# facebookresearch/rela

Measured on AMD Instinct MI355X. Metric: env-steps/s (Ape-X Atari 84x84x4, actor tick + learner grad-step), higher is better.
Workload: dtype f32 (f32 operands as 3 exact bf16 parts on bf16 MFMA; f32-accurate); 1 GPU; Ape-X DQN 80x80 envs/GPU, actor+learner on one MI355X, replay 2^20, B=512, A=18, n=3; device-resident static frames; parallelism=single

## Files before the change

rela_amd/csrc/ffnet.hip:

```cpp
#include <atomic>
#include <cstdlib>

#include "common.h"
#include "gemm_bf16s.h"
#include "gemm_f32emu.h"
#include "gemm_s3.h"
#include "conv_img_s3.h"
#include "conv12_s3.h"
#include "ffnet_layout.h"
#include "ffnet_plan.h"
#include "gemm_lds.h"
#include "param_layout.h"
#include "prof.h"
#define RELA_WEIGHT_PACK_KERNEL
#include "weight_pack.h"

namespace rela_amd {

typedef float f32x4 __attribute__((ext_vector_type(4)));

struct FFNetDev {
  uint4* B1 = nullptr;
  float* b1 = nullptr;
  float *B2 = nullptr, *b2 = nullptr;
// ... 1869 lines not shown
int rela_amd::ffnet_load_extra(rela_ffnet* n, const rela_ffnet_params* p, void* stream_, const ExtraPacks& extra) {
  return ffnet_load_impl(n, p, 1, stream_, extra);
}

int rela_amd::ffnet_load_impl(rela_ffnet* n, const rela_ffnet_params* p, int on_device, void* stream_,
                              const ExtraPacks& extra) {
  RELA_CHECK(n && p, RELA_EINVAL, "rela_ffnet_load: bad arguments");
  hipStream_t s = (hipStream_t)stream_;
  DeviceGuard g(n->device);
  const int A = n->num_action;
  int64_t cnt[kFFNetSegs];
  ffnet_param_counts(A, cnt);
  const float* src[12] = {p->conv1_w, p->conv1_b, p->conv2_w, p->conv2_b, p->conv3_w, p->conv3_b,
                          p->fc_w,    p->fc_b,    p->v_w,     p->v_b,     p->a_w,     p->a_b};
  const float* dv[12];
  float* tmp = nullptr;
  if (int rc = stage_params(src, cnt, 12, on_device, "rela_ffnet_load", &tmp, dv, s)) return rc;
  const uint32_t set = ffnet_pack_set(n->max_rows, n->precision, on_device != 0);
  n->bft_src = ffnet_bft_on_demand(n->max_rows, n->precision, on_device != 0) ? dv[6] : nullptr;
  if (int rc = pack_layouts(n->d, set, dv, 12, A, extra, dv[6], s)) return rc;
  n->packed = set;
  if (int rc = free_staging(tmp, s)) return rc;
  n->loaded = true;
  n->version += 1;
  return RELA_OK;
}

extern "C" int rela_ffnet_forward(const rela_ffnet* n, int N, const uint8_t* s_dev, const float* legal_dev,
                                  float* q_dev, void* ws, int64_t ws_bytes, void* stream_) {
  return rela_amd::ffnet_forward_mode(n, N, s_dev, legal_dev, q_dev, ws, ws_bytes, stream_, kModeNet);
}

int rela_amd::ffnet_forward_mode(const rela_ffnet* n, int N, const uint8_t* s_dev, const float* legal_dev, float* q_dev,
                                 void* ws, int64_t ws_bytes, void* stream_, int mode, int rows_limit) {
  RELA_CHECK(n && n->loaded, RELA_ESTATE, "rela_ffnet_forward: parameters were never loaded");
  const int max_rows = rows_limit < 0 ? n->max_rows : rows_limit;
  RELA_CHECK(N >= 1 && s_dev && legal_dev && q_dev && ws, RELA_EINVAL, "rela_ffnet_forward: bad arguments");
  RELA_CHECK(ws_bytes >= rela_ffnet_workspace_bytes(n, N), RELA_EINVAL,
             "rela_ffnet_forward: workspace of %lld bytes is too small for batch %d", (long long)ws_bytes, N);
  RELA_CHECK(((uintptr_t)s_dev & 15) == 0 && ((uintptr_t)ws & 15) == 0, RELA_EINVAL,
             "rela_ffnet_forward: s_dev and workspace must be 16-byte aligned");
  RELA_CHECK(max_rows <= 0 || N <= max_rows, RELA_EINVAL,
             "rela_ffnet_forward: batch %d on a net whose owner declared at most %d rows", N, max_rows);
  hipStream_t s = (hipStream_t)stream_;
  const FFNetWs w = ffnet_ws(ws, N);
  const FFNetDev& d = n->d;
  const char* const* names = n->prof_names ? n->prof_names : kProfActor;
  const char* name12 = n->prof_names ? "learner_fwd_conv12" : "conv12_fused";
  const FfnetPlan plan = plan_ffnet_forward(mode, n->precision, N, max_rows);
  uint32_t missing = ffnet_plan_reads(plan) & ~n->packed;
  if (missing == lay_bit(kLayBfT) && n->bft_src) {
    if (int rc = pack_one(kLayouts[kLayBfT].kind, n->bft_src, nullptr, n->d.BfT, 0, 0, kLayouts[kLayBfT].elements, s)) return rc;
    n->packed |= lay_bit(kLayBfT);
    missing = 0;
  }
  RELA_CHECK(missing == 0, RELA_ESTATE,
             "rela_ffnet_forward: %d rows in mode %d read layouts (bits 0x%x) the net's last load did not pack (row limit %d)", N,
             plan.precision, missing, n->max_rows);

  uint8_t* rec2 = static_cast<uint8_t*>(ws) + ws_records_offset(N);
  uint8_t* rec3 = rec2 + (int64_t)N * kRec2Bytes;
  TrunkOpts opts;
  opts.keep_f32 = plan.keep_f32;
  opts.leave_a3_records = !plan.unsplit_a3;
  launch_trunk(d, plan.trunk, N, s_dev, w.a1, w.a2, w.a3, rec2, rec3, opts, {names[0], names[1], names[2], name12}, s);

  const uint8_t* a3_records = reinterpret_cast<const uint8_t*>(w.a3);
// ... 8 lines not shown
    case kFcBf16SplitK:
      launch_fc_bf16_splitk(d, a3_records, fc_part_ptr(ws, w.ha, N), w.h, N, names[3], s);
      break;
    case kFcS3:
    case kFcS3SplitK: {
      ProfScope prof(names[3], s);
      note_launch("gemm_s3<fc>");
      const s3::Plan pl = s3::plan<s3::ProbFc>(N, plan.fc == kFcS3SplitK);
      if (pl.slices > 1) {
        float* part = fc_part_ptr(ws, w.ha, N);
        s3::launch<s3::ProbFc, s3::kEpiRaw>(rec3, d.Bfe, d.bf, part, N, s, pl);
        launch_fc_reduce(part, pl.slices, N, d.bf, w.h, s);
      } else {
        s3::launch<s3::ProbFc, s3::kEpiRelu>(rec3, d.Bfe, d.bf, w.h, N, s);
      }
      break;
    }
    case kFcF32SplitK: {
      float* part = fc_part_ptr(ws, w.ha, N);
      ProbFcFwd p{};
      p.M = N, p.N = 512, p.K = 3136;
      p.a3 = w.a3, p.wt = d.BfT, p.part = part;
      gemm::launch_gemm<TileFcSmall>(p, plan.fc_slices, s, names[3]);
      launch_fc_reduce(part, plan.fc_slices, N, d.bf, w.h, s);
      break;
    }
    case kFcF32Gemm: {
      ProfScope prof(names[3], s);
      note_launch("gemm_mfma<GemmFc> (f32)");
      launch_gemm_bm<GemmFc, GemmFc112>(w.a3, nullptr, d.Bf, d.bf, w.h, nullptr, nullptr, N, s);
      break;
    }
  }
  if (plan.trunk == kTrunkS3 && plan.keep_f32) unsplit_s3_a23(rec2, rec3, w.a2, w.a3, N, s);
  {
    ProfScope prof(names[4], s);
    note_launch("heads_duel");
    hipLaunchKernelGGL(heads_duel, dim3(ceil_div(N, kHeadRows)), dim3(256), 0, s, (const float*)w.h, (const float*)d.Bhp,
                       (const float*)d.bh, legal_dev, w.ha, q_dev, N, n->num_action);
  }
  RELA_LAUNCH_CHECK();
  return RELA_OK;
}

namespace rela_amd {
namespace {
__global__ void unsplit_trunk_rows(uint8_t* __restrict__ a1, uint8_t* __restrict__ a2, uint8_t* __restrict__ a3, int rows,
                                   int blocks1, int blocks2) {
  int b = blockIdx.x;
  const int t = threadIdx.x;
  int64_t rec;
  int q, C;
  uint8_t* base;
  bool ok;
  if (b < blocks1) {
    rec = (int64_t)b * 32 + (t >> 3), q = t & 7, C = 32, base = a1, ok = rec < (int64_t)rows * 400;
  } else {
    b -= blocks1;
    base = a2;
    int64_t pixels = (int64_t)rows * 81;
    if (b >= blocks2) b -= blocks2, base = a3, pixels = (int64_t)rows * 49;
    rec = (int64_t)b * 16 + (t >> 4), q = t & 15, C = 64, ok = rec < pixels;
  }
  uint8_t* r = base + (ok ? rec : 0) * (C * 4);
  const uint2 hi = *reinterpret_cast<const uint2*>(r + q * 8), lo = *reinterpret_cast<const uint2*>(r + C * 2 + q * 8);
  float4 v;
  v.x = __uint_as_float(hi.x << 16) + __uint_as_float(lo.x << 16);
// ... 290 lines not shown
```

rela_amd/csrc/ffnet_layout.h:

```cpp
#pragma once
#include <hip/hip_runtime.h>

#include <cstdint>

namespace rela_amd {

constexpr int64_t kA1 = 400 * 32, kA2 = 81 * 64, kA3 = 49 * 64, kH = 512, kHA = 32;
constexpr int64_t kWsFloatsPerSample = kA1 + kA2 + kA3 + kH + kHA;
constexpr int64_t kRec2Bytes = 81 * 384, kRec3Bytes = 49 * 384;

struct FFNetWs {
  float *a1, *a2, *a3, *h, *ha;
};

inline FFNetWs ffnet_ws(void* ws, int N) {
  FFNetWs w;
  w.a1 = static_cast<float*>(ws);
  w.a2 = w.a1 + kA1 * N;
  w.a3 = w.a2 + kA2 * N;
  w.h = w.a3 + kA3 * N;
  w.ha = w.h + kH * N;
  return w;
}

enum { kPermConv2 = 0, kPermConv3 = 1, kPermFc = 2 };
constexpr int kPermFloats[3] = {64 * 512, 64 * 576, 512 * 3136};
__device__ __forceinline__ void permute_weight_at(int mode, int idx, const float* __restrict__ src, float* __restrict__ dst) {
  if (mode == kPermConv2) {
    const int oc = idx >> 9, n = idx & 511, c = n & 31, r = n >> 5;
    dst[idx] = src[((oc * 32 + c) * 4 + (r >> 2)) * 4 + (r & 3)];
  } else if (mode == kPermConv3) {
    const int oc = idx / 576, n = idx - oc * 576, c = n & 63, r = n >> 6;
    dst[idx] = src[((oc * 64 + c) * 3 + r / 3) * 3 + r % 3];
  } else {
    const int u = idx / 3136, n = idx - u * 3136, c = n & 63, pos = n >> 6;
    dst[idx] = src[(size_t)u * 3136 + c * 49 + pos];
  }
}
struct ExtraPacks {
  float *w2p = nullptr, *w3p = nullptr, *wfcp = nullptr;
};
}

#include "../../include/rela_amd.h"
namespace rela_amd {
int ffnet_load_extra(rela_ffnet* n, const rela_ffnet_params* p, void* stream, const ExtraPacks& extra);
int lstmnet_load_extra(rela_lstmnet* n, const rela_lstmnet_params* p, void* stream, const ExtraPacks& extra);
void ffnet_label_as_learner(rela_ffnet* n);
void ffnet_set_max_rows(rela_ffnet* n, int rows);
int ffnet_forward_mode(const rela_ffnet* n, int N, const uint8_t* s_dev, const float* legal_dev, float* q_dev, void* ws,
                       int64_t ws_bytes, void* stream, int mode, int rows_limit = -1);
bool ffnet_learner_forward_ok(const rela_ffnet* on, const rela_ffnet* tg, int B);
int ffnet_learner_forward(const rela_ffnet* on, const rela_ffnet* tg, int B, const uint8_t* s_obs, const uint8_t* s_next,
                          const float* legal, const float* nlegal, float* q_on, float* q_no, float* q_nt, void* ws_on,
                          void* ws_tg, int64_t ws_bytes, hipStream_t s);
int ffnet_learner_unsplit(int B, void* ws_on, hipStream_t s);

int lstmnet_trunk(const rela_lstmnet* n, int N, const uint8_t* s_dev, float* a1, float* a2, float* a3, hipStream_t s,
                  const char* const* names, bool fast = false, bool* a3_records = nullptr, uint8_t* s3_scratch = nullptr,
                  bool keep_f32 = true);
int64_t gate_x3_packed_bytes();
int pack_gate_x3(const float* w_ih_dev, void* dst, bool permuted, hipStream_t s);
int gate_x3_gemm(const uint8_t* a3_records, const void* packed, const float* bias, float* gx, int M, hipStream_t s);
int lstmnet_heads(const rela_lstmnet* n, int N, const float* o, const float* legal, float* ha, float* q, hipStream_t s,
                  const char* name);
int lstmnet_trunk_records(const rela_lstmnet* n, int N, const uint8_t* s_dev, float* a1, float* a2, float* a3, int a1_lo,
                          hipStream_t s, const char* const* names);
int trunk_unsplit_rows(float* a1, float* a2, float* a3, int rows, hipStream_t s);
}
```

rela_amd/csrc/gemm_bf16x3.h:

```cpp
#pragma once
#include <hip/hip_runtime.h>

#include <type_traits>

#include "common.h"
#include "gemm_lds.h"
#include "prof.h"

namespace rela_amd {
namespace gemm3 {

typedef float f32x4 __attribute__((ext_vector_type(4)));
typedef float f32x2 __attribute__((ext_vector_type(2)));
typedef __bf16 bf16x8 __attribute__((ext_vector_type(8)));
typedef __bf16 bf16x2 __attribute__((ext_vector_type(2)));
typedef short s16x4 __attribute__((ext_vector_type(4)));
typedef s16x4 __attribute__((address_space(3))) * lds_s16x4_ptr;

constexpr int kT = 512;
constexpr int BK = 32;

__device__ __forceinline__ int krow(int k) {
  const int g = k >> 3, j = k & 7;
  return j < 4 ? 4 * g + j : 16 + 4 * g + (j - 4);
// ... 62 lines not shown
  }
  const int xcd = blockIdx.x & 7, i = blockIdx.x >> 3;
  if (gm.mode == 1) {
    const int tiles = gm.gx * gm.gy;
    bz = (i / tiles) * 8 + xcd;
    const int t = i % tiles;
    bx = t % gm.gx, by = t / gm.gx;
    return bz < gm.gz;
  }
  bx = (i / gm.gy) * 8 + xcd, by = i % gm.gy, bz = 0;
  return bx < gm.gx;
}

template <class T, class P>
__global__ __launch_bounds__(kT) void gemm_bf16x3(const P p, const GridMap gm) {
  extern __shared__ __attribute__((aligned(16))) uint8_t smem[];
  int bx, by, bz;
  if (!grid_map(gm, bx, by, bz)) return;
  const int tid = threadIdx.x;
  const int wave = tid >> 6, lane = tid & 63;
  const int li = lane & 15, g = lane >> 4;
  const int wm = wave / T::WN, wn = wave % T::WN;
  const int bm0 = by * T::BM, bn0 = bx * T::BN;
  const int nch = (p.K + BK - 1) / BK;
  const int c0 = bz * p.kslice;
  const int c1 = min(nch, c0 + p.kslice);
  constexpr int S = T::S;
  const int r0 = S == 1 ? c0 : 0, r1 = S == 1 ? c1 : (c1 - c0 + S - 1) / S;
  auto kbase = [&](int it, int sub) { return S == 1 ? it * BK : min(c0 + it * S + sub, c1 - 1) * BK; };

  constexpr int D = 4;
  typename P::StageA ra[D][T::A_IT];
  typename P::StageB rb[D][T::B_IT];
  auto gload = [&](int ch, auto set) {
    constexpr int R = decltype(set)::value;
    const int m0 = bm0, n0 = bn0;
#pragma unroll
    for (int j = 0; j < T::A_IT; ++j) {
      const int idx = min(tid + j * kT, T::A_V4 - 1);
      const int sub = idx / T::A_V4C, ic = idx % T::A_V4C;
      const int k0 = kbase(ch, sub);
      if constexpr (T::AMC) {
        const int kr = ic / (T::BM / 4), q = ic % (T::BM / 4);
        ra[R][j] = p.fetchA(k0 + kr, m0 + 4 * q);
      } else {
        const int r = ic >> 3, q = ic & 7;
        ra[R][j] = p.fetchA(m0 + r, k0 + 4 * q);
      }
    }
#pragma unroll
    for (int j = 0; j < T::B_IT; ++j) {
      const int idx = min(tid + j * kT, T::B_V4 - 1);
      const int sub = idx / T::B_V4C, ic = idx % T::B_V4C;
      const int kr = ic / (T::BN / 4), q = ic % (T::BN / 4);
      rb[R][j] = p.fetchB(kbase(ch, sub) + kr, n0 + 4 * q);
    }
  };
  auto sstore = [&](int buf, int ch, auto set) {
    constexpr int R = decltype(set)::value;
    const int z = gemm::store_point();
    const int m0 = bm0 + z, n0 = bn0 + z;
    uint8_t* base = smem + buf * T::BUF;
#pragma unroll
    for (int j = 0; j < T::A_IT; ++j) {
      const int idx = min(tid + j * kT, T::A_V4 - 1);
      const int sub = idx / T::A_V4C, ic = idx % T::A_V4C;
      const int k0 = kbase(ch, sub) + z;
      uint2 hi, mid, lo;
      float4 v;
      int off;
      if constexpr (T::AMC) {
        const int kr = ic / (T::BM / 4), q = ic % (T::BM / 4);
        v = p.fixA(ra[R][j], k0 + kr, m0 + 4 * q);
        off = sub * T::A_CHUNK + krow(kr) * T::LDA + q * 8;
      } else {
        const int r = ic >> 3, q = ic & 7;
        v = p.fixA(ra[R][j], m0 + r, k0 + 4 * q);
        off = sub * T::A_CHUNK + r * T::LDA + q * 8;
      }
      if constexpr (T::PARTS == 3) split4x3(v, hi, mid, lo);
      else split4(v, hi, lo);
      *reinterpret_cast<uint2*>(base + off) = hi;
      if constexpr (T::PARTS == 3) *reinterpret_cast<uint2*>(base + T::A_HALF + off) = mid;
      *reinterpret_cast<uint2*>(base + (T::PARTS - 1) * T::A_HALF + off) = lo;
    }
    uint8_t* bb = base + T::PARTS * T::A_HALF;
#pragma unroll
    for (int j = 0; j < T::B_IT; ++j) {
      const int idx = min(tid + j * kT, T::B_V4 - 1);
      const int sub = idx / T::B_V4C, ic = idx % T::B_V4C;
      const int kr = ic / (T::BN / 4), q = ic % (T::BN / 4);
      uint2 hi, mid, lo;
      const float4 v = p.fixB(rb[R][j], kbase(ch, sub) + z + kr, n0 + 4 * q);
      if constexpr (T::PARTS == 3) split4x3(v, hi, mid, lo);
      else split4(v, hi, lo);
      const int off = sub * T::B_CHUNK + krow(kr) * T::LDB + q * 8;
      *reinterpret_cast<uint2*>(bb + off) = hi;
      if constexpr (T::BPARTS == 3) *reinterpret_cast<uint2*>(bb + T::B_HALF + off) = mid;
      if constexpr (T::BPARTS > 1) *reinterpret_cast<uint2*>(bb + (T::BPARTS - 1) * T::B_HALF + off) = lo;
    }
  };

  const int tr_off = (4 * g + (li >> 2));
  auto frag_tr = [&](const uint8_t* img, int ld, int col0) -> bf16x8 {
    const uint8_t* a0 = img + tr_off * ld + (col0 + 4 * (li & 3)) * 2;
    const s16x4 x = __builtin_amdgcn_ds_read_tr16_b64_v4i16((lds_s16x4_ptr)(a0));
    const s16x4 y = __builtin_amdgcn_ds_read_tr16_b64_v4i16((lds_s16x4_ptr)(a0 + 16 * ld));
    typedef short s16x8 __attribute__((ext_vector_type(8)));
    const s16x8 z = {x[0], x[1], x[2], x[3], y[0], y[1], y[2], y[3]};
    return __builtin_bit_cast(bf16x8, z);
  };
  auto frag_row = [&](const uint8_t* img, int row) -> bf16x8 {
    return __builtin_bit_cast(bf16x8, *reinterpret_cast<const uint4*>(img + row * T::LDA + g * 16));
  };

  f32x4 acc[T::TM][T::TN];
  f32x4 accs[T::PARTS == 3 ? T::TM : 1][T::PARTS == 3 ? T::TN : 1];
#pragma unroll
  for (int t = 0; t < T::TM; ++t)
#pragma unroll
    for (int u = 0; u < T::TN; ++u) {
      acc[t][u] = f32x4{0.f, 0.f, 0.f, 0.f};
      if constexpr (T::PARTS == 3) accs[t][u] = f32x4{0.f, 0.f, 0.f, 0.f};
    }

  auto mma = [&](int buf, int ch, auto full) {
// ... 89 lines not shown
```

rela_amd/csrc/gemm_lds.h:

```cpp
#pragma once
#include <hip/hip_runtime.h>

#include <type_traits>
#include <utility>

#include "common.h"
#include "prof.h"

namespace rela_amd {
namespace gemm {

typedef float f32x4 __attribute__((ext_vector_type(4)));
constexpr int kLT = 512;
constexpr int BK = 32;

__device__ __forceinline__ float4 zero4() { return make_float4(0.f, 0.f, 0.f, 0.f); }
__device__ __forceinline__ float4 ld4(const float* p) { return *reinterpret_cast<const float4*>(p); }
__device__ __forceinline__ float4 keep4(bool in_range, float4 v) {
  return make_float4(in_range ? v.x : 0.f, in_range ? v.y : 0.f, in_range ? v.z : 0.f, in_range ? v.w : 0.f);
}

template <int BM_, int BN_, int WM_, int WN_, bool AMC_, int S_ = 1>
struct TileCfg {
  static constexpr int BM = BM_, BN = BN_, WM = WM_, WN = WN_, S = S_;
  static constexpr bool AMC = AMC_;
  static_assert(S == 1 || S == 2 || S == 4, "stage depth");
  static_assert(WM * WN == 8, "8 wavefronts per block");
  static constexpr int TM = BM / 16 / WM, TN = BN / 16 / WN;
  static_assert(TM >= 1 && TN >= 1, "tile too small for the wave grid");
  static constexpr int LDA = AMC ? BM + 16 : BK + 2;
  static constexpr int A_CHUNK = AMC ? BK * LDA : BM * LDA;
  static constexpr int A_FLOATS = S * A_CHUNK;
  static constexpr int LDB = BN + 16;
  static constexpr int B_CHUNK = BK * LDB;
  static constexpr int B_FLOATS = S * B_CHUNK;
  static constexpr int A_V4C = BM * BK / 4, B_V4C = BN * BK / 4;
  static constexpr int A_V4 = S * A_V4C, B_V4 = S * B_V4C;
  static constexpr int A_IT = (A_V4 + kLT - 1) / kLT, B_IT = (B_V4 + kLT - 1) / kLT;
  static constexpr int LDS_BYTES = 2 * (A_FLOATS + B_FLOATS) * 4;
  static constexpr bool DYN_LDS = LDS_BYTES > 64 * 1024;
};

template <class P, class = void>
struct fold_chunks {
  static constexpr int value = 0;
};
template <class P>
struct fold_chunks<P, std::void_t<decltype(P::kFoldChunks)>> {
  static constexpr int value = P::kFoldChunks;
};

__device__ __forceinline__ int store_point() {
  int z = 0;
  asm volatile("" : "+s"(z));
  return z;
}
template <class F, int... I>
__device__ __forceinline__ void static_for(F&& f, std::integer_sequence<int, I...>) {
  (f(std::integral_constant<int, I>{}), ...);
}
template <int D, class Load, class Store, class Mma>
__device__ __forceinline__ void chunk_ring(int c0, int c1, Load&& gload, Store&& sstore, Mma&& mma) {
  using Sets = std::make_integer_sequence<int, D>;
  static_for([&](auto j) { gload(min(c0 + j.value, c1 - 1), j); }, Sets{});
  sstore(0, c0, std::integral_constant<int, 0>{});
  __syncthreads();
  int base = c0;
  for (; base + D < c1; base += D) {
    static_for(
        [&](auto j) {
          const int cur = base + j.value, buf = (cur - c0) & 1;
          gload(min(cur + D, c1 - 1), j);
          __builtin_amdgcn_sched_barrier(0);
          mma(buf, cur, std::true_type{});
          __builtin_amdgcn_sched_barrier(0);
          sstore(buf ^ 1, cur + 1, std::integral_constant<int, (j.value + 1) % D>{});
          __syncthreads();
          __builtin_amdgcn_sched_barrier(0);
        },
        Sets{});
  }
  static_for(
      [&](auto j) {
// ... 6 lines not shown
      },
      Sets{});
}

constexpr int kRing = 2;

template <class T, class P>
__global__ __launch_bounds__(kLT) void gemm_lds(const P p) {
  constexpr int S = T::S;
  __shared__ __attribute__((aligned(16))) float sA_[2][T::DYN_LDS ? 4 : T::A_FLOATS];
  __shared__ __attribute__((aligned(16))) float sB_[2][T::DYN_LDS ? 4 : T::B_FLOATS];
  extern __shared__ __attribute__((aligned(16))) float gemm_lds_dyn[];
  auto pA = [&](int buf, int off) -> float* {
    if constexpr (T::DYN_LDS) return gemm_lds_dyn + buf * T::A_FLOATS + off;
    else return &sA_[buf][off];
  };
  auto pB = [&](int buf, int off) -> float* {
    if constexpr (T::DYN_LDS) return gemm_lds_dyn + (2 * T::A_FLOATS + buf * T::B_FLOATS) + off;
    else return &sB_[buf][off];
  };
  const int tid = threadIdx.x;
  const int wave = tid >> 6, lane = tid & 63;
  const int li = lane & 15, kk = lane >> 4;
  const int wm = wave / T::WN, wn = wave % T::WN;
  const int bm0 = blockIdx.y * T::BM, bn0 = blockIdx.x * T::BN;
  const int nch = (p.K + BK - 1) / BK;
  const int c0 = blockIdx.z * p.kslice;
  const int c1 = min(nch, c0 + p.kslice);
  const int r0 = S == 1 ? c0 : 0, r1 = S == 1 ? c1 : (c1 - c0 + S - 1) / S;
  auto kbase = [&](int it, int sub) { return S == 1 ? it * BK : min(c0 + it * S + sub, c1 - 1) * BK; };

  typename P::StageA ra[kRing][T::A_IT];
  typename P::StageB rb[kRing][T::B_IT];
  auto gload = [&](int ch, auto set) {
    constexpr int R = decltype(set)::value;
    const int m0 = bm0, n0 = bn0;
#pragma unroll
    for (int j = 0; j < T::A_IT; ++j) {
      const int idx = min(tid + j * kLT, T::A_V4 - 1);
      const int sub = S == 1 ? 0 : idx / T::A_V4C, ic = S == 1 ? idx : idx % T::A_V4C;
      const int k0 = kbase(ch, sub);
      if constexpr (T::AMC) {
        const int kr = ic / (T::BM / 4), q = ic % (T::BM / 4);
        ra[R][j] = p.fetchA(k0 + kr, m0 + 4 * q);
      } else {
        const int r = ic >> 3, q = ic & 7;
        ra[R][j] = p.fetchA(m0 + r, k0 + 4 * q);
      }
    }
#pragma unroll
    for (int j = 0; j < T::B_IT; ++j) {
      const int idx = min(tid + j * kLT, T::B_V4 - 1);
      const int sub = S == 1 ? 0 : idx / T::B_V4C, ic = S == 1 ? idx : idx % T::B_V4C;
      const int kr = ic / (T::BN / 4), q = ic % (T::BN / 4);
      rb[R][j] = p.fetchB(kbase(ch, sub) + kr, n0 + 4 * q);
    }
  };
  auto sstore = [&](int buf, int ch, auto set) {
    constexpr int R = decltype(set)::value;
    const int z = store_point();
    const int k00 = kbase(ch, 0) + z, m0 = bm0 + z, n0 = bn0 + z;
#pragma unroll
    for (int j = 0; j < T::A_IT; ++j) {
      const int idx = min(tid + j * kLT, T::A_V4 - 1);
      const int sub = S == 1 ? 0 : idx / T::A_V4C, ic = S == 1 ? idx : idx % T::A_V4C;
      const int k0 = S == 1 ? k00 : kbase(ch, sub) + z;
      if constexpr (T::AMC) {
        const int kr = ic / (T::BM / 4), q = ic % (T::BM / 4);
        *reinterpret_cast<float4*>(pA(buf, sub * T::A_CHUNK + kr * T::LDA + 4 * q)) = p.fixA(ra[R][j], k0 + kr, m0 + 4 * q);
      } else {
        const int r = ic >> 3, q = ic & 7;
        const float4 v = p.fixA(ra[R][j], m0 + r, k0 + 4 * q);
        float* d = pA(buf, sub * T::A_CHUNK + r * T::LDA + 4 * q);
        *reinterpret_cast<float2*>(d) = make_float2(v.x, v.y);
        *reinterpret_cast<float2*>(d + 2) = make_float2(v.z, v.w);
      }
    }
#pragma unroll
    for (int j = 0; j < T::B_IT; ++j) {
      const int idx = min(tid + j * kLT, T::B_V4 - 1);
      const int sub = S == 1 ? 0 : idx / T::B_V4C, ic = S == 1 ? idx : idx % T::B_V4C;
      const int kr = ic / (T::BN / 4), q = ic % (T::BN / 4);
      *reinterpret_cast<float4*>(pB(buf, sub * T::B_CHUNK + kr * T::LDB + 4 * q)) =
          p.fixB(rb[R][j], (S == 1 ? k00 : kbase(ch, sub) + z) + kr, n0 + 4 * q);
    }
  };

  f32x4 acc[T::TM][T::TN];
#pragma unroll
  for (int t = 0; t < T::TM; ++t)
#pragma unroll
    for (int u = 0; u < T::TN; ++u) acc[t][u] = f32x4{0.f, 0.f, 0.f, 0.f};
  constexpr int FOLD = fold_chunks<P>::value;
  f32x4 tot[FOLD ? T::TM : 1][FOLD ? T::TN : 1];
  if constexpr (FOLD > 0) {
#pragma unroll
    for (int t = 0; t < T::TM; ++t)
#pragma unroll
      for (int u = 0; u < T::TN; ++u) tot[t][u] = f32x4{0.f, 0.f, 0.f, 0.f};
  }

  auto mma = [&](int buf, int ch, auto full) {
    const int left = c1 - c0 - ch * S;
#pragma unroll
    for (int sub = 0; sub < S; ++sub) {
      if (S == 1 || decltype(full)::value || sub < left) {
#pragma unroll
        for (int ks = 0; ks < BK / 4; ++ks) {
          float a[T::TM], b[T::TN];
#pragma unroll
          for (int t = 0; t < T::TM; ++t) {
            const int row = (wm * T::TM + t) * 16 + li;
            a[t] = *pA(buf, sub * T::A_CHUNK + (T::AMC ? (4 * ks + kk) * T::LDA + row : row * T::LDA + 4 * ks + kk));
          }
#pragma unroll
          for (int u = 0; u < T::TN; ++u) b[u] = *pB(buf, sub * T::B_CHUNK + (4 * ks + kk) * T::LDB + (wn * T::TN + u) * 16 + li);
#pragma unroll
// ... 63 lines not shown
```

rela_amd/csrc/learner.hip:

```cpp
#include "learner_common.h"

using namespace rela_amd;

static_assert(sizeof(rela_ffnet_params) == kFFNetSegs * sizeof(float*), "rela_ffnet_params is kFFNetSegs pointers");
struct rela_apex_learner : LearnerCore {
  rela_ffnet *online = nullptr, *target = nullptr;
  float *w2p = nullptr, *w3p = nullptr, *wfcp = nullptr;
  uint8_t *ws_on = nullptr, *ws_tmp = nullptr;
  int64_t ws_bytes = 0;
  float *q = nullptr;
  float *td = nullptr, *d_ha = nullptr, *d_h = nullptr, *d_a3 = nullptr, *d_a2 = nullptr, *d_a1 = nullptr;
  float *part = nullptr;
  float *cpart = nullptr;
  float *s32 = nullptr;
  int pend_B = 0, last_B = 0;
  int pend_rows = 0;
  const uint8_t* pend_obs = nullptr;
  hipStream_t side = nullptr;
  hipEvent_t ev[8] = {nullptr};
  float *part_side = nullptr, *cpart_side = nullptr;
  uint8_t *frag2 = nullptr, *frag3 = nullptr;
};

namespace {
// ... 261 lines not shown
  hipStream_t s = (hipStream_t)stream_;
  DeviceGuard g(l->device);
  const int Bn = batch, A = l->A;
  const uint8_t* obs = static_cast<const uint8_t*>(rows_dev[0]);
  const uint8_t* nobs = static_cast<const uint8_t*>(rows_dev[1]);
  const float* legal = static_cast<const float*>(rows_dev[4]);
  const float* nlegal = static_cast<const float*>(rows_dev[5]);
  const int64_t* act = static_cast<const int64_t*>(rows_dev[6]);
  const float* reward = static_cast<const float*>(rows_dev[7]);
  const float* boot = static_cast<const float*>(rows_dev[9]);
  RELA_CHECK(obs && nobs && legal && nlegal && act && reward && boot, RELA_EINVAL,
             "rela_apex_learner_loss: a batch field is NULL");
  float* q_on = l->q;
  float* q_no = l->q + (size_t)Bn * A;
  float* q_nt = l->q + 2 * (size_t)Bn * A;
  int rc;
  bool unsplit_side = false;
  l->pend_rows = Bn;
  if (rela_ffnet_precision(l->online) == 1 && ffnet_learner_forward_ok(l->online, l->target, Bn)) {
    rc = ffnet_learner_forward(l->online, l->target, Bn, obs, nobs, legal, nlegal, q_on, q_no, q_nt, l->ws_on, l->ws_tmp,
                               l->ws_bytes, s);
    if (rc != RELA_OK) return rc;
    if (l->side) lane_dep(l->ev[0], s, l->side);
    rc = ffnet_learner_unsplit(Bn, l->ws_on, l->side ? l->side : s);
    if (rc != RELA_OK) return rc;
    unsplit_side = l->side != nullptr;
    l->pend_rows = 2 * Bn;
  } else if (rela_ffnet_precision(l->online) == 2 && Bn >= 512 && merge_online_forwards() &&
             nobs == obs + (size_t)Bn * 28224 && nlegal == legal + (size_t)Bn * A) {
    const uint8_t* in2 = obs;
    const float* legal2 = legal;
    rc = rela_ffnet_forward(l->target, Bn, nobs, nlegal, q_nt, l->ws_tmp, l->ws_bytes, s);
    if (rc != RELA_OK) return rc;
    rc = ffnet_forward_mode(l->online, 2 * Bn, in2, legal2, q_on, l->ws_on, l->ws_bytes, s, 3, 2 * l->Bmax);
    if (rc != RELA_OK) return rc;
    l->pend_rows = 2 * Bn;
  } else {
    rc = rela_ffnet_forward(l->online, Bn, nobs, nlegal, q_no, l->ws_tmp, l->ws_bytes, s);
    if (rc != RELA_OK) return rc;
    rc = rela_ffnet_forward(l->target, Bn, nobs, nlegal, q_nt, l->ws_tmp, l->ws_bytes, s);
    if (rc != RELA_OK) return rc;
    rc = ffnet_forward_mode(l->online, Bn, obs, legal, q_on, l->ws_on, l->ws_bytes, s, rela_ffnet_precision(l->online) == 2 ? 3 : 0);
    if (rc != RELA_OK) return rc;
  }
  rc = launch_loss_grad(Bn, A, Bn <= kFusedLossMaxBatch, q_on, q_no, q_nt, nlegal, act, reward, boot, l->gamma_n, l->vr_eps,
                        weight_dev, legal, l->td, priority_dev, l->d_ha, l->loss, s);
  if (rc != RELA_OK) return rc;
  if (loss_dev) RELA_HIP(dev_copy2(loss_dev, l->loss, sizeof(float), nullptr, nullptr, 0, s));
  if (unsplit_side) lane_dep(l->ev[1], l->side, s);
  RELA_LAUNCH_CHECK();
  l->pend_B = l->last_B = Bn;
  l->pend_obs = obs;
  return RELA_OK;
}

extern "C" int rela_apex_learner_grad(rela_apex_learner* l, void* stream_) {
  RELA_CHECK(l && l->loaded && l->pend_B > 0, RELA_ESTATE, "rela_apex_learner_grad: no rela_apex_learner_loss to differentiate");
  hipStream_t s = (hipStream_t)stream_;
  DeviceGuard g(l->device);
  const int Bn = l->pend_B, A = l->A;
  const uint8_t* obs = l->pend_obs;
  l->pend_B = 0;

  const FFNetWs w = ffnet_ws(l->ws_on, l->pend_rows);
  const rela_ffnet_params P = params_at(l, l->P);
  float* Gm[kFFNetSegs];
  for (int i = 0; i < kFFNetSegs; ++i) Gm[i] = l->G + l->off[i];
// ... 177 lines not shown
```

rela_amd/csrc/learner_common.h:

```cpp
#pragma once
#include <cmath>
#include <cstring>
#include <vector>

#include "common.h"
#include "ffnet_layout.h"
#include "gemm_lds.h"
#include "gemm_bf16x3.h"
#include "param_layout.h"
#include "prof.h"
#include "value_rescale.h"
#include "weight_pack.h"
#include "dgrad_conv_bf16.h"
#include "wgrad_conv1_bf16.h"
#include "wgrad_conv2_bf16.h"
#include "wgrad_conv3_bf16.h"

namespace rela_amd {
namespace {

using namespace gemm;

using TileDgrad = TileCfg<128, 64, 4, 2, false>;
using TileWfc = TileCfg<128, 64, 4, 2, true>;
// ... 62 lines not shown
  __device__ float4 fixA(float4 v, int b, int) const { return keep4(b < K, v); }
  __device__ float4 fixB(float4 v, int b, int) const { return keep4(b < K, v); }
  __device__ void store(int, int m, int n, float v) const {
    if (m < A) g_a_w[(size_t)m * 512 + n] = v;
    else if (m == 31) g_v_w[n] = v;
  }
};

struct ProbFcDgrad : ProbBase {
  const float *d_h, *wfcp, *a3;
  float* d_a3;
  __device__ float4 fetchA(int m, int k) const { return ld4(d_h + (size_t)min(m, M - 1) * 512 + k); }
  __device__ float4 fixA(float4 v, int m, int) const { return keep4(m < M, v); }
  __device__ float4 fetchB(int k, int n) const { return ld4(wfcp + (size_t)k * 3136 + n); }
  __device__ void store(int, int m, int n, float v) const {
    const size_t i = (size_t)m * 3136 + n;
    d_a3[i] = a3[i] > 0.f ? v : 0.f;
  }
};

struct ProbFcWgrad : ProbBase {
  const float *d_h, *a3;
  float* g_fc_w;
  __device__ float4 fetchA(int b, int m) const { return ld4(d_h + (size_t)min(b, K - 1) * 512 + m); }
  __device__ float4 fetchB(int b, int n) const { return ld4(a3 + (size_t)min(b, K - 1) * 3136 + n); }
  __device__ float4 fixA(float4 v, int b, int) const { return keep4(b < K, v); }
  __device__ float4 fixB(float4 v, int b, int) const { return keep4(b < K, v); }
  __device__ void store(int, int m, int n, float v) const {
    const int pos = n >> 6, c = n & 63;
    g_fc_w[(size_t)m * 3136 + c * 49 + pos] = v;
  }
};

struct ProbDgrad3 : ProbBase {
  static constexpr int kFoldChunks = 2;
  const float *d_out, *wp, *a2;
  float* d_a2;
  __device__ void tap_pixel(int m, int k, int& b, int& oy, int& ox) const {
    m = min(m, M - 1);
    b = m / 81;
    const int pix = m - b * 81, y = pix / 9, x = pix - y * 9;
    const int tap = k >> 6, kh = tap / 3, kw = tap - kh * 3;
    oy = y - kh, ox = x - kw;
  }
  __device__ float4 fetchA(int m, int k) const {
    int b, oy, ox;
    tap_pixel(m, k, b, oy, ox);
    oy = min(max(oy, 0), 6), ox = min(max(ox, 0), 6);
    return ld4(d_out + ((size_t)b * 49 + oy * 7 + ox) * 64 + (k & 63));
  }
  __device__ float4 fixA(float4 v, int m, int k) const {
    int b, oy, ox;
    tap_pixel(m, k, b, oy, ox);
    return keep4(m < M && (unsigned)oy < 7u && (unsigned)ox < 7u, v);
  }
  __device__ float4 fetchB(int k, int n) const { return ld4(wp + (size_t)(k & 63) * 576 + (k >> 6) * 64 + n); }
  __device__ void store(int, int m, int n, float v) const {
    const size_t i = (size_t)m * 64 + n;
    d_a2[i] = a2[i] > 0.f ? v : 0.f;
  }
};

struct ProbDgrad2 : ProbBase {
  static constexpr int kFoldChunks = 2;
  const float *d_out, *wp, *a1;
  float* d_a1;
  __device__ void tap_pixel(int m, int k, int& b, int& oy, int& ox) const {
    m = min(m, M - 1);
    b = m / 100;
    const int pix = m - b * 100, yh = pix / 10, xh = pix - yh * 10;
    const int t = k >> 6;
    oy = yh - (t >> 1), ox = xh - (t & 1);
  }
  __device__ float4 fetchA(int m, int k) const {
    int b, oy, ox;
    tap_pixel(m, k, b, oy, ox);
    oy = min(max(oy, 0), 8), ox = min(max(ox, 0), 8);
    return ld4(d_out + ((size_t)b * 81 + oy * 9 + ox) * 64 + (k & 63));
  }
  __device__ float4 fixA(float4 v, int m, int k) const {
    int b, oy, ox;
    tap_pixel(m, k, b, oy, ox);
    return keep4(m < M && (unsigned)oy < 9u && (unsigned)ox < 9u, v);
  }
  __device__ float4 fetchB(int k, int n) const {
    const int cls = n >> 5, t = k >> 6;
    const int kh = (t & 2) + (cls >> 1), kw = 2 * (t & 1) + (cls & 1);
    return ld4(wp + (size_t)(k & 63) * 512 + (kh * 4 + kw) * 32 + (n & 31));
  }
  __device__ void store(int, int m, int n, float v) const {
    const int cls = n >> 5;
    const int b = m / 100, pix = m - b * 100;
    const int yh = pix / 10, xh = pix - yh * 10;
    const size_t i = ((size_t)b * 400 + (2 * yh + (cls >> 1)) * 20 + 2 * xh + (cls & 1)) * 32 + (n & 31);
    d_a1[i] = a1[i] > 0.f ? v : 0.f;
  }
};

template <int OC, int CIN, int KH, int KW, int STRIDE, int OH, int OW, int IH, int IW>
struct ProbConvWgrad : ProbBase {
  const float *d_out, *in;
  float* part;
  __device__ float4 fetchA(int k, int m) const { return ld4(d_out + (size_t)min(k, K - 1) * OC + m); }
  __device__ float4 fixA(float4 v, int k, int) const { return keep4(k < K, v); }
  __device__ float4 fixB(float4 v, int k, int) const { return keep4(k < K, v); }
  __device__ float4 fetchB(int k, int n) const {
    k = min(k, K - 1);
    const int b = k / (OH * OW), pos = k - b * (OH * OW);
    const int oy = pos / OW, ox = pos - oy * OW;
    const int r = n / CIN, c = n - r * CIN;
    const int kh = r / KW, kw = r - kh * KW;
    return ld4(in + (((size_t)b * IH + oy * STRIDE + kh) * IW + ox * STRIDE + kw) * CIN + c);
  }
  __device__ void store(int z, int m, int n, float v) const { part[((size_t)z * M + m) * N + n] = v; }
};
using ProbW3 = ProbConvWgrad<64, 64, 3, 3, 1, 7, 7, 9, 9>;
using ProbW2 = ProbConvWgrad<64, 32, 4, 4, 2, 9, 9, 20, 20>;

struct ProbW1 : ProbBase {
  const float* d_out;
  const uint8_t* obs;
  float* part;
  using StageB = uint32_t;
  __device__ float4 fetchA(int k, int m) const { return ld4(d_out + (size_t)min(k, K - 1) * 32 + m); }
  __device__ float4 fixA(float4 v, int k, int) const { return keep4(k < K, v); }
  __device__ uint32_t fetchB(int k, int n) const {
    k = min(k, K - 1);
    const int b = k / 400, pos = k - b * 400;
    const int oy = pos / 20, ox = pos - oy * 20;
    const int c = n >> 6, kh = (n >> 3) & 7, kw = n & 7;
    return *reinterpret_cast<const uint32_t*>(obs + (size_t)b * 28224 + c * 7056 + (oy * 4 + kh) * 84 + ox * 4 + kw);
  }
  __device__ float4 fixB(uint32_t d, int k, int) const {
    return keep4(k < K,
                 make_float4((float)(d & 0xff), (float)((d >> 8) & 0xff), (float)((d >> 16) & 0xff), (float)(d >> 24)));
  }
  __device__ void store(int z, int m, int n, float v) const { part[((size_t)z * M + m) * N + n] = v; }
};


enum { kRedConv1 = 0, kRedConv2 = 1, kRedConv3 = 2 };
__global__ void reduce_splits(const float* __restrict__ part, int splits, int M, int N, int mode,
                              float* __restrict__ out) {
  const int idx = blockIdx.x * blockDim.x + threadIdx.x;
  if (idx >= M * N) return;
  const int m = idx / N, n = idx - m * N;
  float s = 0.f;
#pragma unroll 8
  for (int z = 0; z < splits; ++z) s += part[((size_t)z * M + m) * N + n];
  if (mode == kRedConv1) {
    out[(size_t)m * N + n] = s / 255.0f;
  } else if (mode == kRedConv2) {
    const int c = n & 31, r = n >> 5;
    out[((size_t)(m * 32 + c) * 4 + (r >> 2)) * 4 + (r & 3)] = s;
  } else {
    const int c = n & 63, r = n >> 6;
// ... 266 lines not shown
                            float bc2_sqrt, const float* __restrict__ coef) {
  const int64_t i = (int64_t)blockIdx.x * blockDim.x + threadIdx.x;
  const float cf = coef[1];
  if (i >= n4 || cf < 0.f) return;
  const float4 gv = reinterpret_cast<const float4*>(g)[i];
  float4 av = reinterpret_cast<float4*>(m1)[i], bv = reinterpret_cast<float4*>(m2)[i], pv = reinterpret_cast<float4*>(p)[i];
  auto upd = [&](float gi, float& a, float& b, float& pi) {
    gi = gi * cf;
    a = b1 * a + (1.0f - b1) * gi;
    b = b2 * b + (1.0f - b2) * gi * gi;
    pi -= (lr / bc1) * (a / (sqrtf(b) / bc2_sqrt + eps));
  };
  upd(gv.x, av.x, bv.x, pv.x), upd(gv.y, av.y, bv.y, pv.y), upd(gv.z, av.z, bv.z, pv.z), upd(gv.w, av.w, bv.w, pv.w);
  reinterpret_cast<float4*>(m1)[i] = av;
  reinterpret_cast<float4*>(m2)[i] = bv;
  reinterpret_cast<float4*>(p)[i] = pv;
}


constexpr int kSplitW3 = 28, kSplitW2 = 27, kSplitW1 = 64;
constexpr size_t kTrunkPartFloats = (size_t)w3fast::kMaxBlocks * 64 * 576;
static_assert(kTrunkPartFloats * 4 >= dgfast::kFrag3Bytes && kTrunkPartFloats * 4 >= dgfast::kFrag2Bytes, "frag scratch");
static_assert(kTrunkPartFloats >= (size_t)kSplitW3 * 8 * 64 * 576, "part size (split multiplier up to 8)");
static_assert(kTrunkPartFloats >= (size_t)kSplitW3 * 64 * 576 && kTrunkPartFloats >= (size_t)w1fast::kMaxBlocks * 32 * 256 &&
                  kTrunkPartFloats >= (size_t)w2fast::kMaxBlocks * 64 * 512,
              "part size");
static_assert(kSplitW3 * 64 * 576 >= kSplitW2 * 64 * 512 && kSplitW3 * 64 * 576 >= kSplitW1 * 32 * 256, "part size");
constexpr int kMaxSplitMul = 8;

constexpr int kFastWgradMinFrames = 2048;
constexpr int kTrunkMaxFrames = 32768;
static_assert(((size_t)kTrunkMaxFrames * 100 + TileDgrad2::BM - 1) / TileDgrad2::BM <= 65535 &&
                  ((size_t)kTrunkMaxFrames * 81 + TileDgrad3::BM - 1) / TileDgrad3::BM <= 65535, "grid y extent of the data gradients");
struct TrunkBwd {
  int Bn;
  const uint8_t* obs;
  const float *a1, *a2;
  const float* d_a3;
  float *d_a2, *d_a1;
  float* part;
  float* cpart;
  const float *w2p, *w3p;
  float *g_c1w, *g_c1b, *g_c2w, *g_c2b, *g_c3w, *g_c3b;
  bool fast = false;
  bool emu = false;
  int emu_split_mul[3] = {1, 1, 1};
  int fast_wgrad_min_frames = kFastWgradMinFrames;
  hipStream_t side = nullptr;
  hipEvent_t ev_da3 = nullptr, ev_da2 = nullptr, ev_side = nullptr;
  float *part_side = nullptr, *cpart_side = nullptr;
  const void *frag2 = nullptr, *frag3 = nullptr;
  const float* s32 = nullptr;
  float *g_a_b = nullptr, *g_v_b = nullptr;
  int A = 0;
};
inline void lane_dep(hipEvent_t ev, hipStream_t from, hipStream_t to) {
  (void)hipEventRecord(ev, from);
  (void)hipStreamWaitEvent(to, ev, 0);
}

inline void colsum_multi_launch(ColsumJobs& jobs, float* cpart, hipStream_t s) {
  if (jobs.n == 0) return;
  int maxC = 0;
  size_t off = 0;
  for (int j = 0; j < jobs.n; ++j) {
    jobs.part[j] = cpart + off;
// ... 206 lines not shown
```

Before: 3.765 million env-steps/s.

## Carry incremental gather iterators in conv gradient GEMMs and limit f32 unsplit rows

Adds an optional carried-iterator protocol to the LDS and bf16x3 GEMM mainloops, so problems can keep per-thread gather state across K chunks instead of recomputing divisions and modulos for every fetch. The conv weight-gradient and data-gradient problems (W1, W2, W3, Dgrad2, Dgrad3) opt in, using 32-bit incrementally advanced patch offsets and precomputed row coordinates. Separately, the learner's online forward now unsplits f32 activations only for the first Bn rows rather than all 2*Bn. This adds register pressure and more complex index logic, guarded by 32-bit offset static asserts.

```diff
diff --git a/rela_amd/csrc/ffnet.hip b/rela_amd/csrc/ffnet.hip
--- a/rela_amd/csrc/ffnet.hip
+++ b/rela_amd/csrc/ffnet.hip
@@ -1925,7 +1925,7 @@
 }
 
 int rela_amd::ffnet_forward_mode(const rela_ffnet* n, int N, const uint8_t* s_dev, const float* legal_dev, float* q_dev,
-                                 void* ws, int64_t ws_bytes, void* stream_, int mode, int rows_limit) {
+                                 void* ws, int64_t ws_bytes, void* stream_, int mode, int rows_limit, int f32_rows) {
   RELA_CHECK(n && n->loaded, RELA_ESTATE, "rela_ffnet_forward: parameters were never loaded");
   const int max_rows = rows_limit < 0 ? n->max_rows : rows_limit;
   RELA_CHECK(N >= 1 && s_dev && legal_dev && q_dev && ws, RELA_EINVAL, "rela_ffnet_forward: bad arguments");
@@ -2000,7 +2000,7 @@
       break;
     }
   }
-  if (plan.trunk == kTrunkS3 && plan.keep_f32) unsplit_s3_a23(rec2, rec3, w.a2, w.a3, N, s);
+  if (plan.trunk == kTrunkS3 && plan.keep_f32) unsplit_s3_a23(rec2, rec3, w.a2, w.a3, f32_rows < 0 ? N : std::min(f32_rows, N), s);
   {
     ProfScope prof(names[4], s);
     note_launch("heads_duel");
diff --git a/rela_amd/csrc/ffnet_layout.h b/rela_amd/csrc/ffnet_layout.h
--- a/rela_amd/csrc/ffnet_layout.h
+++ b/rela_amd/csrc/ffnet_layout.h
@@ -49,7 +49,7 @@
 void ffnet_label_as_learner(rela_ffnet* n);
 void ffnet_set_max_rows(rela_ffnet* n, int rows);
 int ffnet_forward_mode(const rela_ffnet* n, int N, const uint8_t* s_dev, const float* legal_dev, float* q_dev, void* ws,
-                       int64_t ws_bytes, void* stream, int mode, int rows_limit = -1);
+                       int64_t ws_bytes, void* stream, int mode, int rows_limit = -1, int f32_rows = -1);
 bool ffnet_learner_forward_ok(const rela_ffnet* on, const rela_ffnet* tg, int B);
 int ffnet_learner_forward(const rela_ffnet* on, const rela_ffnet* tg, int B, const uint8_t* s_obs, const uint8_t* s_next,
                           const float* legal, const float* nlegal, float* q_on, float* q_no, float* q_nt, void* ws_on,
diff --git a/rela_amd/csrc/gemm_bf16x3.h b/rela_amd/csrc/gemm_bf16x3.h
--- a/rela_amd/csrc/gemm_bf16x3.h
+++ b/rela_amd/csrc/gemm_bf16x3.h
@@ -118,15 +118,41 @@
   constexpr int D = 4;
   typename P::StageA ra[D][T::A_IT];
   typename P::StageB rb[D][T::B_IT];
+  constexpr bool CA = gemm::carries_a<P>::value, CB = gemm::carries_b<P>::value;
+  typename gemm::carry_a_state<P, CA>::type ita[T::A_IT];
+  typename gemm::carry_b_state<P, CB>::type itb[T::B_IT];
+  int held = r0;
+  if constexpr (CA) {
+#pragma unroll
+    for (int j = 0; j < T::A_IT; ++j) {
+      const int idx = min(tid + j * kT, T::A_V4 - 1);
+      const int sub = idx / T::A_V4C, ic = idx % T::A_V4C;
+      if constexpr (T::AMC) ita[j] = p.initA(kbase(r0, sub) + ic / (T::BM / 4), bm0 + 4 * (ic % (T::BM / 4)));
+      else ita[j] = p.initA(bm0 + (ic >> 3), kbase(r0, sub) + 4 * (ic & 7));
+    }
+  }
+  if constexpr (CB) {
+#pragma unroll
+    for (int j = 0; j < T::B_IT; ++j) {
+      const int idx = min(tid + j * kT, T::B_V4 - 1);
+      const int sub = idx / T::B_V4C, ic = idx % T::B_V4C;
+      itb[j] = p.initB(kbase(r0, sub) + ic / (T::BN / 4), bn0 + 4 * (ic % (T::BN / 4)));
+    }
+  }
   auto gload = [&](int ch, auto set) {
     constexpr int R = decltype(set)::value;
     const int m0 = bm0, n0 = bn0;
+    const bool moved = ch > held;
+    held = ch;
 #pragma unroll
     for (int j = 0; j < T::A_IT; ++j) {
       const int idx = min(tid + j * kT, T::A_V4 - 1);
       const int sub = idx / T::A_V4C, ic = idx % T::A_V4C;
       const int k0 = kbase(ch, sub);
-      if constexpr (T::AMC) {
+      if constexpr (CA) {
+        p.template advA<S * BK>(ita[j], moved && (S == 1 || c0 + ch * S + gemm::carry_sub<T::A_V4C, T::A_V4, kT>(tid, j) < c1));
+        ra[R][j] = p.fetchA(ita[j], k0);
+      } else if constexpr (T::AMC) {
         const int kr = ic / (T::BM / 4), q = ic % (T::BM / 4);
         ra[R][j] = p.fetchA(k0 + kr, m0 + 4 * q);
       } else {
@@ -139,7 +165,12 @@
       const int idx = min(tid + j * kT, T::B_V4 - 1);
       const int sub = idx / T::B_V4C, ic = idx % T::B_V4C;
       const int kr = ic / (T::BN / 4), q = ic % (T::BN / 4);
-      rb[R][j] = p.fetchB(kbase(ch, sub) + kr, n0 + 4 * q);
+      if constexpr (CB) {
+        p.template advB<S * BK>(itb[j], moved && (S == 1 || c0 + ch * S + gemm::carry_sub<T::B_V4C, T::B_V4, kT>(tid, j) < c1));
+        rb[R][j] = p.fetchB(itb[j], kbase(ch, sub));
+      } else {
+        rb[R][j] = p.fetchB(kbase(ch, sub) + kr, n0 + 4 * q);
+      }
     }
   };
   auto sstore = [&](int buf, int ch, auto set) {
@@ -157,11 +188,13 @@
       int off;
       if constexpr (T::AMC) {
         const int kr = ic / (T::BM / 4), q = ic % (T::BM / 4);
-        v = p.fixA(ra[R][j], k0 + kr, m0 + 4 * q);
+        if constexpr (CA) v = p.fixA(ra[R][j], ita[j], k0, k0 + kr, m0 + 4 * q);
+        else v = p.fixA(ra[R][j], k0 + kr, m0 + 4 * q);
         off = sub * T::A_CHUNK + krow(kr) * T::LDA + q * 8;
       } else {
         const int r = ic >> 3, q = ic & 7;
-        v = p.fixA(ra[R][j], m0 + r, k0 + 4 * q);
+        if constexpr (CA) v = p.fixA(ra[R][j], ita[j], k0, m0 + r, k0 + 4 * q);
+        else v = p.fixA(ra[R][j], m0 + r, k0 + 4 * q);
         off = sub * T::A_CHUNK + r * T::LDA + q * 8;
       }
       if constexpr (T::PARTS == 3) split4x3(v, hi, mid, lo);
@@ -177,7 +210,10 @@
       const int sub = idx / T::B_V4C, ic = idx % T::B_V4C;
       const int kr = ic / (T::BN / 4), q = ic % (T::BN / 4);
       uint2 hi, mid, lo;
-      const float4 v = p.fixB(rb[R][j], kbase(ch, sub) + z + kr, n0 + 4 * q);
+      const int k0 = kbase(ch, sub) + z;
+      float4 v;
+      if constexpr (CB) v = p.fixB(rb[R][j], itb[j], k0, k0 + kr, n0 + 4 * q);
+      else v = p.fixB(rb[R][j], k0 + kr, n0 + 4 * q);
       if constexpr (T::PARTS == 3) split4x3(v, hi, mid, lo);
       else split4(v, hi, lo);
       const int off = sub * T::B_CHUNK + krow(kr) * T::LDB + q * 8;
diff --git a/rela_amd/csrc/gemm_lds.h b/rela_amd/csrc/gemm_lds.h
--- a/rela_amd/csrc/gemm_lds.h
+++ b/rela_amd/csrc/gemm_lds.h
@@ -49,6 +49,37 @@
 struct fold_chunks<P, std::void_t<decltype(P::kFoldChunks)>> {
   static constexpr int value = P::kFoldChunks;
 };
+
+template <class P, class = void>
+struct carries_a : std::false_type {};
+template <class P>
+struct carries_a<P, std::void_t<decltype(P::kCarryA)>> : std::bool_constant<P::kCarryA> {};
+template <class P, class = void>
+struct carries_b : std::false_type {};
+template <class P>
+struct carries_b<P, std::void_t<decltype(P::kCarryB)>> : std::bool_constant<P::kCarryB> {};
+struct NoCarry {};
+template <class P, bool ON>
+struct carry_a_state {
+  using type = NoCarry;
+};
+template <class P>
+struct carry_a_state<P, true> {
+  using type = typename P::ItA;
+};
+template <class P, bool ON>
+struct carry_b_state {
+  using type = NoCarry;
+};
+template <class P>
+struct carry_b_state<P, true> {
+  using type = typename P::ItB;
+};
+template <int V4C, int V4, int THREADS>
+__device__ __forceinline__ int carry_sub(int tid, int j) {
+  if constexpr (V4C % THREADS == 0) return (j * THREADS) / V4C;
+  else return min(tid + j * THREADS, V4 - 1) / V4C;
+}
 
 __device__ __forceinline__ int store_point() {
   int z = 0;
@@ -121,15 +152,41 @@
 
   typename P::StageA ra[kRing][T::A_IT];
   typename P::StageB rb[kRing][T::B_IT];
+  constexpr bool CA = carries_a<P>::value, CB = carries_b<P>::value;
+  typename carry_a_state<P, CA>::type ita[T::A_IT];
+  typename carry_b_state<P, CB>::type itb[T::B_IT];
+  int held = r0;
+  if constexpr (CA) {
+#pragma unroll
+    for (int j = 0; j < T::A_IT; ++j) {
+      const int idx = min(tid + j * kLT, T::A_V4 - 1);
+      const int sub = S == 1 ? 0 : idx / T::A_V4C, ic = S == 1 ? idx : idx % T::A_V4C;
+      if constexpr (T::AMC) ita[j] = p.initA(kbase(r0, sub) + ic / (T::BM / 4), bm0 + 4 * (ic % (T::BM / 4)));
+      else ita[j] = p.initA(bm0 + (ic >> 3), kbase(r0, sub) + 4 * (ic & 7));
+    }
+  }
+  if constexpr (CB) {
+#pragma unroll
+    for (int j = 0; j < T::B_IT; ++j) {
+      const int idx = min(tid + j * kLT, T::B_V4 - 1);
+      const int sub = S == 1 ? 0 : idx / T::B_V4C, ic = S == 1 ? idx : idx % T::B_V4C;
+      itb[j] = p.initB(kbase(r0, sub) + ic / (T::BN / 4), bn0 + 4 * (ic % (T::BN / 4)));
+    }
+  }
   auto gload = [&](int ch, auto set) {
     constexpr int R = decltype(set)::value;
     const int m0 = bm0, n0 = bn0;
+    const bool moved = ch > held;
+    held = ch;
 #pragma unroll
     for (int j = 0; j < T::A_IT; ++j) {
       const int idx = min(tid + j * kLT, T::A_V4 - 1);
       const int sub = S == 1 ? 0 : idx / T::A_V4C, ic = S == 1 ? idx : idx % T::A_V4C;
       const int k0 = kbase(ch, sub);
-      if constexpr (T::AMC) {
+      if constexpr (CA) {
+        p.template advA<S * BK>(ita[j], moved && (S == 1 || c0 + ch * S + carry_sub<T::A_V4C, T::A_V4, kLT>(tid, j) < c1));
+        ra[R][j] = p.fetchA(ita[j], k0);
+      } else if constexpr (T::AMC) {
         const int kr = ic / (T::BM / 4), q = ic % (T::BM / 4);
         ra[R][j] = p.fetchA(k0 + kr, m0 + 4 * q);
       } else {
@@ -142,7 +199,12 @@
       const int idx = min(tid + j * kLT, T::B_V4 - 1);
       const int sub = S == 1 ? 0 : idx / T::B_V4C, ic = S == 1 ? idx : idx % T::B_V4C;
       const int kr = ic / (T::BN / 4), q = ic % (T::BN / 4);
-      rb[R][j] = p.fetchB(kbase(ch, sub) + kr, n0 + 4 * q);
+      if constexpr (CB) {
+        p.template advB<S * BK>(itb[j], moved && (S == 1 || c0 + ch * S + carry_sub<T::B_V4C, T::B_V4, kLT>(tid, j) < c1));
+        rb[R][j] = p.fetchB(itb[j], kbase(ch, sub));
+      } else {
+        rb[R][j] = p.fetchB(kbase(ch, sub) + kr, n0 + 4 * q);
+      }
     }
   };
   auto sstore = [&](int buf, int ch, auto set) {
@@ -156,10 +218,15 @@
       const int k0 = S == 1 ? k00 : kbase(ch, sub) + z;
       if constexpr (T::AMC) {
         const int kr = ic / (T::BM / 4), q = ic % (T::BM / 4);
-        *reinterpret_cast<float4*>(pA(buf, sub * T::A_CHUNK + kr * T::LDA + 4 * q)) = p.fixA(ra[R][j], k0 + kr, m0 + 4 * q);
+        float4 v;
+        if constexpr (CA) v = p.fixA(ra[R][j], ita[j], k0, k0 + kr, m0 + 4 * q);
+        else v = p.fixA(ra[R][j], k0 + kr, m0 + 4 * q);
+        *reinterpret_cast<float4*>(pA(buf, sub * T::A_CHUNK + kr * T::LDA + 4 * q)) = v;
       } else {
         const int r = ic >> 3, q = ic & 7;
-        const float4 v = p.fixA(ra[R][j], m0 + r, k0 + 4 * q);
+        float4 v;
+        if constexpr (CA) v = p.fixA(ra[R][j], ita[j], k0, m0 + r, k0 + 4 * q);
+        else v = p.fixA(ra[R][j], m0 + r, k0 + 4 * q);
         float* d = pA(buf, sub * T::A_CHUNK + r * T::LDA + 4 * q);
         *reinterpret_cast<float2*>(d) = make_float2(v.x, v.y);
         *reinterpret_cast<float2*>(d + 2) = make_float2(v.z, v.w);
@@ -170,8 +237,11 @@
       const int idx = min(tid + j * kLT, T::B_V4 - 1);
       const int sub = S == 1 ? 0 : idx / T::B_V4C, ic = S == 1 ? idx : idx % T::B_V4C;
       const int kr = ic / (T::BN / 4), q = ic % (T::BN / 4);
-      *reinterpret_cast<float4*>(pB(buf, sub * T::B_CHUNK + kr * T::LDB + 4 * q)) =
-          p.fixB(rb[R][j], (S == 1 ? k00 : kbase(ch, sub) + z) + kr, n0 + 4 * q);
+      const int k0 = S == 1 ? k00 : kbase(ch, sub) + z;
+      float4 v;
+      if constexpr (CB) v = p.fixB(rb[R][j], itb[j], k0, k0 + kr, n0 + 4 * q);
+      else v = p.fixB(rb[R][j], k0 + kr, n0 + 4 * q);
+      *reinterpret_cast<float4*>(pB(buf, sub * T::B_CHUNK + kr * T::LDB + 4 * q)) = v;
     }
   };
 
diff --git a/rela_amd/csrc/learner.hip b/rela_amd/csrc/learner.hip
--- a/rela_amd/csrc/learner.hip
+++ b/rela_amd/csrc/learner.hip
@@ -317,7 +317,7 @@
     const float* legal2 = legal;
     rc = rela_ffnet_forward(l->target, Bn, nobs, nlegal, q_nt, l->ws_tmp, l->ws_bytes, s);
     if (rc != RELA_OK) return rc;
-    rc = ffnet_forward_mode(l->online, 2 * Bn, in2, legal2, q_on, l->ws_on, l->ws_bytes, s, 3, 2 * l->Bmax);
+    rc = ffnet_forward_mode(l->online, 2 * Bn, in2, legal2, q_on, l->ws_on, l->ws_bytes, s, 3, 2 * l->Bmax, Bn);
     if (rc != RELA_OK) return rc;
     l->pend_rows = 2 * Bn;
   } else {
diff --git a/rela_amd/csrc/learner_common.h b/rela_amd/csrc/learner_common.h
--- a/rela_amd/csrc/learner_common.h
+++ b/rela_amd/csrc/learner_common.h
@@ -118,9 +118,44 @@
   }
 };
 
+#ifndef RELA_CARRY_DGRAD3
+#define RELA_CARRY_DGRAD3 1
+#endif
+#ifndef RELA_CARRY_DGRAD2
+#define RELA_CARRY_DGRAD2 1
+#endif
+#ifndef RELA_CARRY_WCONV
+#define RELA_CARRY_WCONV 1
+#endif
+#ifndef RELA_CARRY_W1
+#define RELA_CARRY_W1 1
+#endif
+struct DgradRow {
+  uint32_t base;
+  int y, x;
+  static constexpr int kNoRow = -64;
+};
+
 struct ProbDgrad3 : ProbBase {
   static constexpr int kFoldChunks = 2;
+  static constexpr bool kCarryA = RELA_CARRY_DGRAD3;
+  using ItA = DgradRow;
   const float *d_out, *wp, *a2;
+  __device__ ItA initA(int m, int k) const {
+    const int mc = min(m, M - 1), b = mc / 81, pix = mc - b * 81, y = pix / 9;
+    return ItA{(uint32_t)b * (49 * 64) + (k & 31), m < M ? y : ItA::kNoRow, pix - y * 9};
+  }
+  template <int DK>
+  __device__ void advA(ItA&, bool) const {}
+  __device__ float4 fetchA(const ItA& it, int k0) const {
+    const int tap = k0 >> 6, kh = tap / 3, kw = tap - kh * 3;
+    const int oy = min(max(it.y - kh, 0), 6), ox = min(max(it.x - kw, 0), 6);
+    return ld4(d_out + (it.base + (uint32_t)((oy * 7 + ox) * 64 + (k0 & 32))));
+  }
+  __device__ float4 fixA(float4 v, const ItA& it, int k0, int, int) const {
+    const int tap = k0 >> 6, kh = tap / 3, kw = tap - kh * 3;
+    return keep4((unsigned)(it.y - kh) < 7u && (unsigned)(it.x - kw) < 7u, v);
+  }
   float* d_a2;
   __device__ void tap_pixel(int m, int k, int& b, int& oy, int& ox) const {
     m = min(m, M - 1);
@@ -149,8 +184,25 @@
 
 struct ProbDgrad2 : ProbBase {
   static constexpr int kFoldChunks = 2;
+  static constexpr bool kCarryA = RELA_CARRY_DGRAD2;
+  using ItA = DgradRow;
   const float *d_out, *wp, *a1;
   float* d_a1;
+  __device__ ItA initA(int m, int k) const {
+    const int mc = min(m, M - 1), b = mc / 100, pix = mc - b * 100, yh = pix / 10;
+    return ItA{(uint32_t)b * (81 * 64) + (k & 31), m < M ? yh : ItA::kNoRow, pix - yh * 10};
+  }
+  template <int DK>
+  __device__ void advA(ItA&, bool) const {}
+  __device__ float4 fetchA(const ItA& it, int k0) const {
+    const int t = k0 >> 6;
+    const int oy = min(max(it.y - (t >> 1), 0), 8), ox = min(max(it.x - (t & 1), 0), 8);
+    return ld4(d_out + (it.base + (uint32_t)((oy * 9 + ox) * 64 + (k0 & 32))));
+  }
+  __device__ float4 fixA(float4 v, const ItA& it, int k0, int, int) const {
+    const int t = k0 >> 6;
+    return keep4((unsigned)(it.y - (t >> 1)) < 9u && (unsigned)(it.x - (t & 1)) < 9u, v);
+  }
   __device__ void tap_pixel(int m, int k, int& b, int& oy, int& ox) const {
     m = min(m, M - 1);
     b = m / 100;
@@ -183,10 +235,50 @@
   }
 };
 
+template <int OH, int OW, int FRAME, int ROW, int COL>
+struct PatchWalk {
+  uint32_t off;
+  int rpos, rx;
+  __device__ void init(int k, uint32_t fixed) {
+    const int b = k / (OH * OW), pos = k - b * (OH * OW);
+    const int oy = pos / OW, ox = pos - oy * OW;
+    rpos = OH * OW - 1 - pos, rx = OW - 1 - ox;
+    off = (uint32_t)b * FRAME + oy * ROW + ox * COL + fixed;
+  }
+  template <int DK>
+  __device__ void advance(bool step) {
+    static_assert(DK > 0 && DK < OH * OW, "one frame wrap per advance");
+    static_assert(FRAME < (1 << 23) && ROW < (1 << 23), "24-bit multiplies");
+    constexpr int DY = DK / OW, DX = DK % OW;
+    const int tx = rx - (step ? DX : 0), tp = rpos - (step ? DK : 0);
+    const int mx = tx >> 31, mp = tp >> 31;
+    rx = __mul24(mx, -OW) + tx, rpos = __mul24(mp, -(OH * OW)) + tp;
+    off += step ? DY * ROW + DX * COL : 0;
+    off += (uint32_t)__mul24(mx, -(ROW - OW * COL));
+    off += (uint32_t)__mul24(mp, -(FRAME - OH * ROW));
+  }
+  __device__ uint32_t clamped(int K, int width) const { return min(off, (uint32_t)(K / (OH * OW)) * FRAME - width); }
+};
+
 template <int OC, int CIN, int KH, int KW, int STRIDE, int OH, int OW, int IH, int IW>
 struct ProbConvWgrad : ProbBase {
+  static constexpr bool kCarryB = RELA_CARRY_WCONV;
+  using ItB = PatchWalk<OH, OW, IH * IW * CIN, STRIDE * IW * CIN, STRIDE * CIN>;
   const float *d_out, *in;
   float* part;
+  __device__ ItB initB(int k, int n) const {
+    const int r = n / CIN, c = n - r * CIN;
+    const int kh = r / KW, kw = r - kh * KW;
+    ItB it;
+    it.init(k, (kh * IW + kw) * CIN + c);
+    return it;
+  }
+  template <int DK>
+  __device__ void advB(ItB& it, bool step) const {
+    it.template advance<DK>(step);
+  }
+  __device__ float4 fetchB(const ItB& it, int) const { return ld4(in + it.clamped(K, 4)); }
+  __device__ float4 fixB(float4 v, const ItB&, int, int k, int) const { return keep4(k < K, v); }
   __device__ float4 fetchA(int k, int m) const { return ld4(d_out + (size_t)min(k, K - 1) * OC + m); }
   __device__ float4 fixA(float4 v, int k, int) const { return keep4(k < K, v); }
   __device__ float4 fixB(float4 v, int k, int) const { return keep4(k < K, v); }
@@ -208,6 +300,22 @@
   const uint8_t* obs;
   float* part;
   using StageB = uint32_t;
+  static constexpr bool kCarryB = RELA_CARRY_W1;
+  using ItB = PatchWalk<20, 20, 28224, 4 * 84, 4>;
+  __device__ ItB initB(int k, int n) const {
+    const int c = n >> 6, kh = (n >> 3) & 7, kw = n & 7;
+    ItB it;
+    it.init(k, c * 7056 + kh * 84 + kw);
+    return it;
+  }
+  template <int DK>
+  __device__ void advB(ItB& it, bool step) const {
+    it.template advance<DK>(step);
+  }
+  __device__ uint32_t fetchB(const ItB& it, int) const {
+    return *reinterpret_cast<const uint32_t*>(obs + it.clamped(K, 4));
+  }
+  __device__ float4 fixB(uint32_t d, const ItB&, int, int k, int n) const { return fixB(d, k, n); }
   __device__ float4 fetchA(int k, int m) const { return ld4(d_out + (size_t)min(k, K - 1) * 32 + m); }
   __device__ float4 fixA(float4 v, int k, int) const { return keep4(k < K, v); }
   __device__ uint32_t fetchB(int k, int n) const {
@@ -540,6 +648,8 @@
 constexpr int kTrunkMaxFrames = 32768;
 static_assert(((size_t)kTrunkMaxFrames * 100 + TileDgrad2::BM - 1) / TileDgrad2::BM <= 65535 &&
                   ((size_t)kTrunkMaxFrames * 81 + TileDgrad3::BM - 1) / TileDgrad3::BM <= 65535, "grid y extent of the data gradients");
+static_assert((uint64_t)kTrunkMaxFrames * 28224 < (1ull << 32) && (uint64_t)kTrunkMaxFrames * 20 * 20 * 32 < (1ull << 32),
+              "32-bit element offsets of the carried gathers (PatchWalk, DgradRow): the largest tensors are obs and a1");
 struct TrunkBwd {
   int Bn;
   const uint8_t* obs;
```

Result: no change. 3.744 million env-steps/s (-0.6%).
